# uthree/tinyvc

Measured on AMD Instinct MI355X. Metric: audio-samples/sec (16 kHz) end-to-end VC, higher is better.
Workload: dtype f32 (fp32 in / out / accumulate; channel contractions as two-term fp16 splits on v_mfma_f32_32x32x16_f16: 22-bit significands, three part-products per fp32 product)

## Files before the change

tinyvc_amd/csrc/api.hip:

```cpp
#include <atomic>
#include <cmath>
#include <mutex>

#include <cstdlib>

#include "knn_blob.h"
#include "tvc_common.h"

using namespace tvc;

static std::mutex g_blob_mu;
static std::map<const void*, int64_t> g_blobs;
constexpr size_t kMaxBlobRecords = 4096;
static void blob_record(const void* p, int64_t N) {
    std::lock_guard<std::mutex> lk(g_blob_mu);
    if (g_blobs.size() >= kMaxBlobRecords && !g_blobs.count(p)) g_blobs.clear();
    g_blobs[p] = N;
}
static void blob_forget(const void* p) {
    std::lock_guard<std::mutex> lk(g_blob_mu);
    g_blobs.erase(p);
}
static int blob_check(tvc_ctx* ctx, hipStream_t s, const void* p, int64_t N, const char* what) {
    {
// ... 12 lines not shown
        return fail(ctx, TVC_ERR_HIP, "%s: cannot read the prepared index's header", what);
    const int64_t n = ((int64_t)(unsigned)h[BLOB_W_N_HI] << 32) | (unsigned)h[BLOB_W_N_LO];
    if (h[BLOB_W_MAGIC] != BLOB_MAGIC || (h[BLOB_W_KIND] != KIND_F32 && h[BLOB_W_KIND] != KIND_F16))
        return fail(ctx, TVC_ERR_ARG, "%s: `prepared` is not a blob of tvc_knn_prepare_index_f32 / _f16", what);
    if (h[BLOB_W_VERSION] != tvc::kBlobVersion)
        return fail(ctx, TVC_ERR_ARG, "%s: the prepared index has format version %d, this library writes and reads version %d: prepare it again", what, h[BLOB_W_VERSION], tvc::kBlobVersion);
    if (n != N) return fail(ctx, TVC_ERR_ARG, "%s: this blob was prepared for N = %lld index vectors, the call says N = %lld", what, (long long)n, (long long)N);
    blob_record(p, N);
    return 0;
}

static int draw_under_capture(tvc_ctx* ctx, hipStream_t s, const float* noise_angle, const char* what) {
    if (noise_angle) return 0;
    hipStreamCaptureStatus cap = hipStreamCaptureStatusNone;
    if (hipStreamIsCapturing(s, &cap) == hipSuccess && cap != hipStreamCaptureStatusNone)
        return fail(ctx, TVC_ERR_STATE, "%s: noise_angle = NULL inside a stream capture would replay ONE seed's phases on every graph launch; pass noise_angle", what);
    return 0;
}

extern "C" {

int tvc_version(void) { return TVC_ABI_VERSION; }

int tvc_ctx_create(int hip_device, tvc_ctx** out) {
    if (!out) return TVC_ERR_ARG;
    *out = nullptr;
    int count = 0;
    if (hipGetDeviceCount(&count) != hipSuccess || hip_device < 0 || hip_device >= count) return TVC_ERR_HIP;
    tvc_ctx* c = new tvc_ctx();
    c->device = hip_device;
    {
        ArenaBuilder ab;
        pack_constants(c, &ab);
        if (hipSetDevice(hip_device) != hipSuccess ||
            hipMalloc((void**)&c->const_arena, ab.buf.size() * sizeof(float)) != hipSuccess ||
            hipMemcpy(c->const_arena, ab.buf.data(), ab.buf.size() * sizeof(float), hipMemcpyHostToDevice) != hipSuccess) {
            if (c->const_arena) (void)hipFree(c->const_arena);
            delete c;
            return TVC_ERR_HIP;
        }
        ab.resolve(c->const_arena);
    }
    if (hipDeviceGetAttribute(&c->ncu, hipDeviceAttributeMultiprocessorCount, hip_device) != hipSuccess) {
        tvc_ctx_destroy(c);
        return TVC_ERR_HIP;
    }
    int prio_least = 0, prio_greatest = 0;
    (void)hipDeviceGetStreamPriorityRange(&prio_least, &prio_greatest);
    if (hipStreamCreateWithPriority(&c->side, hipStreamNonBlocking, prio_least) != hipSuccess ||
        hipEventCreateWithFlags(&c->ev_fork, hipEventDisableTiming) != hipSuccess ||
        hipEventCreateWithFlags(&c->ev_join, hipEventDisableTiming) != hipSuccess ||
        hipEventCreateWithFlags(&c->ev_fork2, hipEventDisableTiming) != hipSuccess ||
        hipEventCreateWithFlags(&c->ev_join2, hipEventDisableTiming) != hipSuccess ||
        hipEventCreateWithFlags(&c->ev_amps, hipEventDisableTiming) != hipSuccess) {
        tvc_ctx_destroy(c);
        return TVC_ERR_HIP;
    }
    *out = c;
    return TVC_OK;
}

void tvc_ctx_destroy(tvc_ctx* ctx) {
    if (!ctx) return;
    (void)hipSetDevice(ctx->device);
    for (auto& r : ctx->regions) {
        if (r.a) (void)hipEventDestroy(r.a);
        if (r.b) (void)hipEventDestroy(r.b);
    }
    for (auto e : ctx->event_pool) (void)hipEventDestroy(e);
    if (ctx->ev_fork) (void)hipEventDestroy(ctx->ev_fork);
    if (ctx->ev_join) (void)hipEventDestroy(ctx->ev_join);
    if (ctx->ev_fork2) (void)hipEventDestroy(ctx->ev_fork2);
    if (ctx->ev_join2) (void)hipEventDestroy(ctx->ev_join2);
    if (ctx->ev_amps) (void)hipEventDestroy(ctx->ev_amps);
    if (ctx->side) (void)hipStreamDestroy(ctx->side);
    frontdoor_release(ctx);
    if (ctx->arena) (void)hipFree(ctx->arena);
    if (ctx->const_arena) (void)hipFree(ctx->const_arena);
    delete ctx;
}

const char* tvc_last_error(const tvc_ctx* ctx) { return ctx ? ctx->err : "null ctx"; }

int tvc_load_tensor(tvc_ctx* ctx, const char* key, const float* host_data, const int64_t* shape, int ndim) {
    if (!ctx || !key || !host_data || !shape || ndim < 1 || ndim > 4) return fail(ctx, TVC_ERR_ARG, "tvc_load_tensor: bad argument");
    size_t n = 1;
    HostTensor t;
    for (int i = 0; i < ndim; ++i) {
        if (shape[i] <= 0) return fail(ctx, TVC_ERR_ARG, "tvc_load_tensor(%s): bad shape", key);
        n *= (size_t)shape[i];
        t.shape.push_back(shape[i]);
    }
    t.data.assign(host_data, host_data + n);
    ctx->host[key] = std::move(t);
    ctx->enc_ready = ctx->dec_ready = false;
    return TVC_OK;
}

int tvc_set_pitch_table(tvc_ctx* ctx, const float* host_freqs, int n) {
    if (!ctx || !host_freqs || n != kPitchClasses) return fail(ctx, TVC_ERR_ARG, "pitch table must have %d entries", kPitchClasses);
    ctx->pitch_table.assign(host_freqs, host_freqs + n);
    ctx->enc_ready = ctx->dec_ready = false;
    return TVC_OK;
}

int tvc_finalize_weights(tvc_ctx* ctx) {
    if (!ctx) return TVC_ERR_ARG;
    ctx->enc_ready = ctx->dec_ready = false;
    ArenaBuilder ab;
    std::string missing_enc, missing_dec;
    pack_checkpoint(ctx, &ab, &missing_enc, &missing_dec);
    snprintf(ctx->enc_missing, sizeof(ctx->enc_missing), "%s", missing_enc.c_str());
    snprintf(ctx->dec_missing, sizeof(ctx->dec_missing), "%s", missing_dec.c_str());
    if (!missing_enc.empty() && !missing_dec.empty())
        return fail(ctx, TVC_ERR_STATE, "no complete checkpoint: encoder lacks %s; decoder lacks %s", missing_enc.c_str(), missing_dec.c_str());

    TVC_HIP(ctx, hipSetDevice(ctx->device));
    if (ctx->arena) {
        TVC_HIP(ctx, hipFree(ctx->arena));
        ctx->arena = nullptr;
    }
    ctx->arena_floats = ab.buf.size();
    TVC_HIP(ctx, hipMalloc((void**)&ctx->arena, ctx->arena_floats * sizeof(float)));
    TVC_HIP(ctx, hipMemcpy(ctx->arena, ab.buf.data(), ctx->arena_floats * sizeof(float), hipMemcpyHostToDevice));
    ab.resolve(ctx->arena);
    ctx->enc_ready = missing_enc.empty();
    ctx->dec_ready = missing_dec.empty();
// ... 1240 lines not shown
```

tinyvc_amd/csrc/decoder.hip:

```cpp
#include "conv3s.h"
#include "conv_s2.h"
#include "film_s2.h"
#include "gemm_s2.h"
#include "small_kernels.h"
#include "tvc_common.h"

namespace tvc {


__device__ __forceinline__ float div24k(float x) {
    const float r = 1.0f / 24000.0f;
    const float q0 = __fmul_rn(x, r);
    return fmaf(fmaf(-q0, 24000.0f, x), r, q0);
}

__device__ __forceinline__ double wave_incl_scan(double v, int lane) {
#pragma unroll
    for (int o = 1; o < 64; o <<= 1) {
        double u = __shfl_up(v, o);
        if (lane >= o) v += u;
    }
    return v;
}

// ... 171 lines not shown
    return launch_check(ctx, "harm_sums");
}

int run_dsp(tvc_ctx* ctx, hipStream_t s, Ws& ws, const float* f0, const float* amps, const float* kern, const float* angle, uint64_t seed, float* source, int B, int T,
            float* smax, double* csum, const DspFork* fk) {
    const long L = (long)T * kHop;
    if (!csum) csum = ws.get<double>((size_t)B * kHarm * T);
    float* frames = ws.get<float>((size_t)B * T * kNfft);
    const int NB = ctx->rag ? ctx->rag->B : B;
    const int Tg = ctx->rag ? ctx->rag->Tlong : T;
    float* smax_own = smax ? nullptr : ws.get<float>((size_t)NB);
    if (ws.dry) return 0;
    if (!smax) {
        smax = smax_own;
        TVC_HIP(ctx, hipMemsetAsync(smax, 0, (size_t)NB * sizeof(float), s));
    }
    RagDev rg;
    TVC_CHECK(rag_view(ctx, s, 1, 0, &rg, nullptr));
    const float scale_size = (float)T / (float)L;
    const float scale_amp = (float)(1.0 / (double)kHop);
    hipStream_t sh = s;
    if (fk) {
        sh = fk->side;
        TVC_HIP(ctx, hipStreamWaitEvent(sh, fk->amps_ready, 0));
    } else {
        TVC_CHECK(run_harm_sums(ctx, s, f0, csum, B, T));
    }
    hipLaunchKernelGGL(harm_synth_kernel, dim3((Tg + 3) / 4, NB), dim3(256), 0, sh, f0, amps, csum, source, T, scale_size, scale_amp, rg);
    TVC_CHECK(run_amax_rows(ctx, sh, amps, B, kHarm, T, smax));
    TVC_CHECK(run_noise_ifft(ctx, s, kern, angle, seed, frames, B, T, ctx->rag && angle));
    hipLaunchKernelGGL(noise_ola_kernel, dim3(grid_for((long)Tg * kHop / 4, 256, NB >= 32 ? 16 : 512 / NB), NB), dim3(256), 0, s, frames, source, B, T, smax, rg);
    return launch_check(ctx, "dsp");
}

static int plain_conv(tvc_ctx* ctx, hipStream_t s, const PackedW& w, const float* x, int B, int Cin, int len, int dil, float* y, const BfpSlots& bfp, int lin = 0,
                      float lscale = 0.f) {
    int rc = 0;
    if ((lin > 0 ? conv_s2_try<true>(&rc, ctx, s, w, x, B, Cin, len, dil, y, bfp, lin, lscale) : conv_s2_try<false>(&rc, ctx, s, w, x, B, Cin, len, dil, y, bfp)))
        return rc;
    if (lin > 0)
        return conv3s_launch<true, C3EpiBias<false>, false, true>(ctx, s, w, x, B, Cin, len, dil, C3EpiBias<false>{y, w.bias, nullptr, w.M, len}, bfp, nullptr, nullptr,
                                                                   nullptr, 0, lin, lscale);
    return conv3s_launch<true>(ctx, s, w, x, B, Cin, len, dil, C3EpiBias<false>{y, w.bias, nullptr, w.M, len}, bfp);
}

static int film_conv(tvc_ctx* ctx, hipStream_t s, const PackedW& w, const PackedW& fw, const FilmU& fu, const float* h, const float* cond, int B, int C, int len, int dil,
                     float* out, const float* bsc, const float* bsh, const float* res, int res_lin, float res_scale, const BfpSlots& bfp) {
    int rc = 0;
    if (rag_min_len(ctx, len) >= FS2::BN && film_s2_try(&rc, ctx, s, fu, h, cond, B, C, len, dil, out, res, res_lin, res_scale, bfp)) return rc;
    return conv3s_launch<true, C3EpiFilmFused, true>(ctx, s, w, h, B, C, len, dil, C3EpiFilmFused{out, w.bias, bsc, bsh, res, C, len, res_lin, res_scale}, bfp, &fw, &fw,
                                                     cond, C);
}

static int conv_film_half(tvc_ctx* ctx, hipStream_t s, const PackedW& ca, const PackedW& cb, const PackedW& fw, const FilmU& fu, const float* x, int lin, float lscale,
                          int da, int db, float* h, const float* cond, int B, int C, int len, float* out, const float* bsc, const float* bsh, const float* res,
                          int res_lin, float res_scale, const float* ma_in, float* mh, const float* mcond, float* mout) {
    const bool pre = rag_min_len(ctx, len) >= FS2::BN && fu.img && fu.C == C && fu.hb_w > 0.f && C % 96 == 0 && C <= 384 && ma_in && mcond && res && db >= 1 && db <= FS2::MAXD &&
                     (long)C * len * 4 < (1L << 32) && (res_lin <= 0 || (long)C * res_lin * 4 < (1L << 32));
    if (pre) {
        int rc = 0;
        const BfpSlots in{ma_in, nullptr, nullptr};
        const bool ok = lin > 0 ? conv_s2_try<true, true>(&rc, ctx, s, ca, x, B, C, len, da, h, in, lin, lscale, fu.hb_w, fu.hb_b)
                                : conv_s2_try<false, true>(&rc, ctx, s, ca, x, B, C, len, da, h, in, 0, 0.f, fu.hb_w, fu.hb_b);
        if (ok) {
            TVC_CHECK(rc);
            if (!film_s2_try(&rc, ctx, s, fu, h, cond, B, C, len, db, out, res, res_lin, res_scale, BfpSlots{ma_in, mcond, mout}, true, fu.hb_w, fu.hb_b))
                return fail(ctx, TVC_ERR_STATE, "filter_net: the FiLM conv refused the pre-split operand its producer wrote");
            return rc;
        }
    }
    TVC_CHECK(plain_conv(ctx, s, ca, x, B, C, len, da, h, BfpSlots{ma_in, nullptr, mh}, lin, lscale));
    return film_conv(ctx, s, cb, fw, fu, h, cond, B, C, len, db, out, bsc, bsh, res, res_lin, res_scale, BfpSlots{mh, mcond, mout});
}

static __global__ void g8_to_planar_kernel(const float* __restrict__ x, float* __restrict__ y, long B, long l, int C) {
    const long n = B * C * l;
    for (long i = blockIdx.x * (long)blockDim.x + threadIdx.x; i < n; i += (long)gridDim.x * blockDim.x) {
        const long t = i % l, bc = i / l, c = bc % C, b = bc / C;
        y[i] = x[((b * (C / 8) + c / 8) * l + t) * 8 + (c & 7)];
    }
}

static int filter_input_gemm(tvc_ctx* ctx, hipStream_t s, const float* content, const float* f0, float* x, int B, int T, const float* cmax) {
    EpiSumCond ep{x, ctx->flt_content_in.bias, nullptr, f0, nullptr, nullptr, ctx->flt_f_w, ctx->flt_f_b, 384, T, B * T};
    int rc = 0;
    if (!gemm_s2_try(&rc, ctx, s, ctx->flt_content_in, content, B, kSslDim, T, 0, ep, cmax)) rc = gemm_s_launch<2, 4, 2>(ctx, s, ctx->flt_content_in, content, B, kSslDim, T, 0, ep, cmax);
    return rc;
}

int run_filter(tvc_ctx* ctx, hipStream_t s, Ws& ws, const float* content, const float* f0,
               const float* energy, const float* source, float* wave, int B, int T, const FilterTaps* taps, const float* cmax, const float* smax, float* zeroed_slots, bool x_slot_set,
               float* x_pre, bool x_pre_filled) {
    const long L = (long)T * kHop;
    static const int ch[5] = {384, 192, 96, 48, 24};
    const long len_dn[5] = {L, L / 5, L / 20, L / 80, L / 240};
    float* skip[5];
    for (int i = 0; i < 5; ++i) skip[i] = ws.get<float>((size_t)B * ch[4 - i] * len_dn[i]);
    float* x = x_pre ? x_pre : ws.get<float>((size_t)B * ch[0] * T);
    float* xi_pre[5] = {nullptr, nullptr, nullptr, nullptr, nullptr};
    for (int i = 1; i <= 4; ++i) xi_pre[i] = ws.get<float>((size_t)B * ctx->downs[i - 1].cin * len_dn[i]);
    for (int i = 1; i < 4; ++i)
        if (len_dn[i] % ctx->downs[i].factor != 0 || (ctx->downs[i].factor == 4 && len_dn[i] % 4 != 0))
            return fail(ctx, TVC_ERR_ARG, "filter_net: level lengths must divide by the next Downsample factor");

    enum { S_CONTENT = 0, S_SRC, S_X, S_SKIP0, S_DH1 = S_SKIP0 + 5, S_DH2 = S_DH1 + 4, S_UHA = S_DH2 + 4, S_UX1 = S_UHA + 5, S_UHB = S_UX1 + 5, S_UXU = S_UHB + 5,
           S_LEV = S_UXU + 5, S_COUNT = S_LEV + 5 };
    const int NB = ctx->rag ? ctx->rag->B : B;
    static_assert(S_COUNT == kFilterSlots && S_X == kFilterSlotX, "tvc_common.h kFilterSlots / kFilterSlotX");
    float* slots = zeroed_slots ? zeroed_slots : ws.get<float>((size_t)S_COUNT * NB);
    auto slot = [&](int i) { return slots + (size_t)i * NB; };

    if (!ws.dry) {
        ProfScope ps(ctx, s, ws, "filter.in+down0");
        if (!zeroed_slots) TVC_HIP(ctx, hipMemsetAsync(slots, 0, (size_t)S_COUNT * NB * sizeof(float), s));
        if (!cmax) {
            TVC_CHECK(run_amax_rows(ctx, s, content, B, kSslDim, T, slot(S_CONTENT)));
            cmax = slot(S_CONTENT);
        }
        if (!smax) {
            TVC_CHECK(run_amax_rows(ctx, s, source, B, 16, L, slot(S_SRC)));
            TVC_CHECK(run_amax_rows(ctx, s, energy, B, 1, L, slot(S_SRC)));
            smax = slot(S_SRC);
        }
        if (!x_pre_filled) TVC_CHECK(filter_input_gemm(ctx, s, content, f0, x, B, T, cmax));
        if (!(zeroed_slots && x_slot_set)) TVC_CHECK(run_slot_affine(ctx, s, slot(S_X), cmax, 1, ctx->flt_in_bw, ctx->flt_in_bb, NB));
        TVC_CHECK(run_down0_split(ctx, s, ctx->flt_down0s, source, energy, skip[0], taps ? taps->skips[0] : nullptr, xi_pre[1], B, (int)L, smax, slot(S_SKIP0)));
    }
    for (int i = 1; i <= 4; ++i) {
        const DownW& d = ctx->downs[i - 1];
        const int len = (int)len_dn[i];
        size_t mk = ws.mark();
        float* xi = xi_pre[i];
        float* h1 = d.cin == 24 ? nullptr : ws.get<float>((size_t)B * d.cin * len);
        float* h2 = d.cin == 24 ? nullptr : ws.get<float>((size_t)B * d.cin * len);
        if (!ws.dry) {
            static const char* names[4] = {"filter.down1", "filter.down2", "filter.down3", "filter.down4"};
            ProfScope ps(ctx, s, ws, names[i - 1]);
            float* y2 = i < 4 ? xi_pre[i + 1] : nullptr;
            const int f2 = i < 4 ? ctx->downs[i].factor : 0;
            const float* mxi = slot(S_SKIP0 + i - 1);
            float *mh1 = slot(S_DH1 + i - 1), *mh2 = slot(S_DH2 + i - 1), *mout = slot(S_SKIP0 + i);
            if (d.cin == 24) {
                TVC_CHECK(run_down24_fused(ctx, s, d, xi, skip[i], y2, B, len, mxi, mout));
            } else {
                if (d.cin == 48) {
                    TVC_CHECK(run_conv48_pair(ctx, s, d.c1, d.c2, xi, 0, 0.f, nullptr, nullptr, nullptr, nullptr, h2, B, len, 1, 2, mxi, nullptr, mh2));
                } else {
                    TVC_CHECK(plain_conv(ctx, s, d.c1, xi, B, d.cin, len, 1, h1, BfpSlots{mxi, nullptr, mh1}));
                    TVC_CHECK(plain_conv(ctx, s, d.c2, h1, B, d.cin, len, 2, h2, BfpSlots{mh1, nullptr, mh2}));
                }
                TVC_CHECK((conv3s_launch<true, C3EpiBiasResConv>(ctx, s, d.c3, h2, B, d.cin, len, 4,
                                                                 C3EpiBiasResConv{{skip[i], d.c3res_bias, nullptr, d.cout, len, y2, f2}},
                                                                 BfpSlots{mh2, mxi, mout}, &d.res, nullptr, xi, d.cin)));
            }
        }
        ws.release(mk);
    }
    float* xlev[5];
    {
        long l = T;
        for (int i = 0; i < 5; ++i) {
            l *= ctx->ups[i].factor;
            xlev[i] = ws.get<float>((size_t)B * ctx->ups[i].cout * l);
        }
    }
    long len = T;
    const float* mx_in = slot(S_X);
    for (int i = 0; i < 5; ++i) {
        const UpW& u = ctx->ups[i];
        const int lin = (int)len;
        len *= u.factor;
        const int lo = (int)len, C = u.cin, nc = B * lo;
        const float* cond = skip[4 - i];
        const float* mcond = slot(S_SKIP0 + 4 - i);
        size_t mk = ws.mark();
        float* xu = ws.get<float>((size_t)B * C * lo);
        float* h = ws.get<float>((size_t)B * C * lo);
        float* x1 = ws.get<float>((size_t)B * C * lo);
        if (!ws.dry && C == 24) {
            ProfScope ps(ctx, s, ws, "filter.up4+out");
            TVC_CHECK(run_up24_split(ctx, s, u, x, cond, ctx->down0_bw, ctx->down0_bb, x1, wave, B, lo, mx_in, smax, slot(S_UX1 + i)));
        } else if (!ws.dry) {
            static const char* names[4] = {"filter.up0", "filter.up1", "filter.up2", "filter.up3"};
            ProfScope ps(ctx, s, ws, names[i]);
            const float lscale = (float)(1.0 / (double)u.factor);
            for (int half = 0; half < 2; ++half) {
                const PackedW& ca = half ? u.c3 : u.c1;
                const PackedW& cb = half ? u.c4 : u.c2;
                const PackedW& fw = half ? u.film2 : u.film1;
                const float* bsc = fw.bias;
                const float* bsh = fw.bias + C;
                const int da = half ? 9 : 1, db = half ? 27 : 3;
                float* xout = half ? xu : x1;
                const float* ma_in = half ? slot(S_UX1 + i) : mx_in;
                float* mh = slot((half ? S_UHB : S_UHA) + i);
                float* mout = slot((half ? S_UXU : S_UX1) + i);
                if (C == 48) {
                    if (half == 0) {
                        TVC_CHECK(run_conv48_pair(ctx, s, ca, cb, x, lin, lscale, &fw, bsc, bsh, cond, xout, B, lo, da, db, ma_in, mcond, mout));
                    } else {
                        TVC_CHECK(run_conv48s(ctx, s, ca, x1, nullptr, nullptr, nullptr, nullptr, nullptr, h, B, lo, da, ma_in, nullptr, mh));
                        TVC_CHECK(run_conv48s(ctx, s, cb, h, &fw, bsc, bsh, cond, x1, nullptr, B, lo, db, mh, mcond, slot(S_LEV + i), &u.c5, xlev[i]));
                    }
                } else if (half == 0) {
                    TVC_CHECK(conv_film_half(ctx, s, ca, cb, fw, u.fu1, x, lin, lscale, da, db, h, cond, B, C, lo, xout, bsc, bsh, x, lin, lscale, ma_in, mh, mcond, mout));
                } else {
                    TVC_CHECK(conv_film_half(ctx, s, ca, cb, fw, u.fu2, x1, 0, 0.f, da, db, h, cond, B, C, lo, xout, bsc, bsh, x1, 0, 0.f, ma_in, mh, mcond, mout));
                }
            }
            if (C != 48) {
                EpiBias<ACT_NONE, false> ep{xlev[i], u.c5.bias, nullptr, u.cout, lo, nc, (long)u.cout * lo, 0, slot(S_LEV + i), slot(S_UXU + i), u.c5_bw, u.c5_bb, NB};
                if (u.cout == 48) {
                    EpiBiasG8 eg{xlev[i], u.c5.bias, u.cout, lo, nc, slot(S_LEV + i), slot(S_UXU + i), u.c5_bw, u.c5_bb, NB};
                    TVC_CHECK((gemm_s_launch<2, 4, 2>(ctx, s, u.c5, xu, B, C, lo, 0, eg, slot(S_UXU + i))));
                } else if (u.c5.MT6 % 3 == 0) TVC_CHECK((gemm_s_launch<3, 4, 1>(ctx, s, u.c5, xu, B, C, lo, 0, ep, slot(S_UXU + i))));
                else TVC_CHECK((gemm_s_launch<2, 4, 2>(ctx, s, u.c5, xu, B, C, lo, 0, ep, slot(S_UXU + i))));
            }
        }
        ws.release(mk);
        x = xlev[i];
        mx_in = slot(S_LEV + i);
    }
    if (!ws.dry && taps) {
        for (int i = 1; i < 5; ++i)
            if (taps->skips[i] && i == 1)
                hipLaunchKernelGGL(g8_to_planar_kernel, dim3(grid_for((long)B * 48 * len_dn[1])), dim3(256), 0, s, skip[1], taps->skips[1], (long)B, len_dn[1], 48);
            else if (taps->skips[i])
                TVC_HIP(ctx, hipMemcpyAsync(taps->skips[i], skip[i], (size_t)B * ch[4 - i] * len_dn[i] * sizeof(float), hipMemcpyDeviceToDevice, s));
        long l = T;
        for (int i = 0; i < 4; ++i) {
            l *= ctx->ups[i].factor;
            if (taps->ups[i] && ctx->ups[i].cout <= 48)
                hipLaunchKernelGGL(g8_to_planar_kernel, dim3(grid_for((long)B * ctx->ups[i].cout * l)), dim3(256), 0, s, xlev[i], taps->ups[i], (long)B, l, ctx->ups[i].cout);
            else if (taps->ups[i])
                TVC_HIP(ctx, hipMemcpyAsync(taps->ups[i], xlev[i], (size_t)B * ctx->ups[i].cout * l * sizeof(float), hipMemcpyDeviceToDevice, s));
        }
    }
    return ws.dry ? 0 : launch_check(ctx, "filter_net");
}

int run_decoder(tvc_ctx* ctx, hipStream_t s, Ws& ws, const float* content, const float* f0,
                const float* energy, const float* angle, uint64_t seed, float* wave, float* amps_out,
                float* kernel_out, float* source_out, int B, int T, const float* content_bound, const float* energy_bound,
                int content_bound_stride) {
    const long L = (long)T * kHop;
    float* amps = amps_out ? amps_out : ws.get<float>((size_t)B * kHarm * T);
    float* kern = kernel_out ? kernel_out : ws.get<float>((size_t)B * kBins * T);
    float* source = source_out ? source_out : ws.get<float>((size_t)B * 16 * L);
    const int NB = ctx->rag ? ctx->rag->B : B;
    float* cmax = ws.get<float>((size_t)(3 + kFilterSlots) * NB);
    float* smax = cmax + NB;
    float* xmax = smax + NB;
    float* fslots = xmax + NB;
    float* x0 = ws.get<float>((size_t)B * 384 * T);
    double* csum = ws.get<double>((size_t)B * kHarm * T);
    if (!ws.dry) {
        TVC_CHECK(run_slot_prep(ctx, s, cmax, (3 + kFilterSlots) * NB, content_bound ? cmax : nullptr, content_bound, content_bound_stride, 1.f, 0.f, energy_bound ? smax : nullptr,
                                energy_bound, 1, 1.f, 0.f, content_bound ? fslots + (size_t)kFilterSlotX * NB : nullptr, ctx->flt_in_bw, ctx->flt_in_bb,
                                NB));
        if (!content_bound) TVC_CHECK(run_amax_rows(ctx, s, content, B, kSslDim, T, cmax));
        if (!energy_bound) TVC_CHECK(run_amax_rows(ctx, s, energy, B, 1, L, smax));
    }
    SideFork fk(ctx, s);
    if (wave) TVC_CHECK(fk.fork(ws, ctx->ev_fork2, ctx->ev_join2));
    if (fk.forked()) {
        TVC_CHECK(run_harm_sums(ctx, fk.side, f0, csum, B, T));
        ProfScope ps(ctx, fk.side, ws, "filter_net.input@side");
        TVC_CHECK(filter_input_gemm(ctx, fk.side, content, f0, x0, B, T, cmax));
    }
    size_t mk = ws.mark();
    {
        ProfScope ps(ctx, s, ws, "source_net");
        TVC_CHECK(run_source_net(ctx, s, ws, content, f0, energy, amps, kern, B, T, cmax, xmax, fk.forked() ? ctx->ev_amps : nullptr));
    }
    ws.release(mk);
    if (!wave && !source_out) return 0;
    {
        ProfScope ps(ctx, s, ws, "dsp");
        const DspFork df{fk.side, ctx->ev_amps};
        TVC_CHECK(run_dsp(ctx, s, ws, f0, amps, kern, angle, seed, source, B, T, smax, csum, fk.forked() ? &df : nullptr));
        TVC_CHECK(fk.join());
    }
    ws.release(mk);
    if (!wave) return 0;
    ProfScope ps(ctx, s, ws, "filter_net");
    TVC_CHECK(run_filter(ctx, s, ws, content, f0, energy, source, wave, B, T, nullptr, cmax, smax, fslots, content_bound != nullptr, x0, fk.forked()));
    ws.release(mk);
    return 0;
}

}
```

tinyvc_amd/csrc/tvc_common.h:

```cpp
#pragma once
#include <hip/hip_runtime.h>

#include <atomic>
#include <cstdarg>
#include <cstdint>
#include <cstdio>
#include <cstring>
#include <map>
#include <string>
#include <vector>

#include "../../include/tinyvc_hip.h"
#include "ragged.h"

namespace tvc {

constexpr int kSampleRate = 24000;
constexpr int kNfft = 1920;
constexpr int kHop = 480;
constexpr int kBins = 961;
constexpr int kSslDim = 768;
constexpr int kSslCh = 384;
constexpr int kPitchCh = 128;
constexpr int kPitchClasses = 512;
// ... 52 lines not shown
    const float* s24c1 = nullptr;
    const float* s24c2 = nullptr;
    const float* s24c3r = nullptr;
    float b1_w = 0.f, b1_b = 0.f, b2_w = 0.f, b2_b = 0.f;
    int cin = 0, cout = 0, factor = 1;
};
struct FilmU {
    static constexpr int TAB_BIAS = 0, TAB_SCALE = 1, TAB_BSC = 2, TAB_BSH = 3, TAB_SSC = 4, TAB_SSH = 5;
    const float* img = nullptr;
    const float* tab = nullptr;
    int C = 0;
    float hb_w = 0.f, hb_b = 0.f;
};
struct UpW {
    PackedW c1, c2, c3, c4, c5, film1, film2;
    FilmU fu1, fu2;
    const float* s24a = nullptr;
    const float* s24b = nullptr;
    float c5_bw = 0.f, c5_bb = 0.f;
    int cin = 0, cout = 0, factor = 1;
};

struct HostTensor {
    std::vector<float> data;
    std::vector<int64_t> shape;
};

struct ArenaBuilder {
    std::vector<float> buf;
    std::vector<std::pair<const float**, size_t>> fix;
    size_t put(const float** slot, const float* v, size_t n);
    size_t put(const float** slot, const std::vector<float>& v) { return put(slot, v.data(), v.size()); }
    void resolve(const float* arena) const {
        for (auto& f : fix) *f.first = arena + f.second;
    }
};

}

struct tvc_prof_region {
    std::string name;
    hipEvent_t a = nullptr, b = nullptr;
};

struct tvc_ctx {
    int device = 0;
    int ncu = 0;
    int profiling = 0;
    std::vector<tvc_prof_region> regions;
    std::vector<hipEvent_t> event_pool;
    hipStream_t side = nullptr;
    hipEvent_t ev_fork = nullptr, ev_join = nullptr;
    hipEvent_t ev_fork2 = nullptr, ev_join2 = nullptr, ev_amps = nullptr;
    tvc::RagHost* rag = nullptr;
    int rag_batch_frames = 0;
    int index_assign_chunk = 0;
    bool enc_ready = false, dec_ready = false;
    char enc_missing[160] = {0}, dec_missing[160] = {0};
    std::map<std::string, tvc::HostTensor> host;
    std::vector<float> pitch_table;
    float* arena = nullptr;
    float* const_arena = nullptr;
    size_t arena_floats = 0;
    char err[512] = {0};

    const float* fft_tw960 = nullptr;
    const float* fft_tw1920 = nullptr;
    const float* fft_hann = nullptr;
    const float* pitch_freq = nullptr;
    const float* sola_part = nullptr;
    const float* dn_win = nullptr;
    const float* dn_tw320 = nullptr;
    const float* dn_tw640 = nullptr;

    tvc::PackedW enc_in;
    const float* ssl_ln_g = nullptr;
    const float* ssl_ln_b = nullptr;
    const float* pit_ln_g = nullptr;
    const float* pit_ln_b = nullptr;
    tvc::ConvNeXtW ssl_mid[6], pit_mid[4], src_mid[3];
    tvc::PackedW ssl_out, pit_out;
    tvc::PackedW src_content_in, src_to_amps, src_to_kernel;
    const float* src_e_w = nullptr;
    const float* src_e_b = nullptr;
    const float* src_f_w = nullptr;
    const float* src_f_b = nullptr;
    tvc::PackedW flt_content_in;
    const float* flt_down0s = nullptr;
    float down0_bw = 0.f, down0_bb = 0.f;
    float flt_in_bw = 0.f, flt_in_bb = 0.f;
    const float* flt_f_w = nullptr;
    const float* flt_f_b = nullptr;
    tvc::DownW downs[4];
    tvc::UpW ups[5];
};

namespace tvc {

inline int fail(tvc_ctx* ctx, int code, const char* fmt, ...) {
    if (ctx) {
        va_list ap;
        va_start(ap, fmt);
        vsnprintf(ctx->err, sizeof(ctx->err), fmt, ap);
        va_end(ap);
    }
    return code;
// ... 22 lines not shown
    T* get(size_t n) {
        size_t bytes = (n * sizeof(T) + 255) & ~size_t(255);
        size_t o = off;
        off += bytes;
        if (off > peak) peak = off;
        if (dry) return (T*)(uintptr_t)256;
        return (T*)(base + o);
    }
    size_t mark() const { return off; }
    void release(size_t m) { off = m; }
};

struct ProfScope {
    tvc_ctx* ctx;
    hipStream_t s;
    int idx = -1;
    ProfScope(tvc_ctx* c, hipStream_t st, const Ws& ws, const char* name) : ctx(c), s(st) {
        if (!c || !c->profiling || ws.dry) return;
        if (c->profiling == 2 && std::strncmp(name, "filter_net", 10) != 0) return;
        tvc_prof_region r;
        r.name = name;
        auto take = [&](hipEvent_t* e) {
            if (!c->event_pool.empty()) {
                *e = c->event_pool.back();
                c->event_pool.pop_back();
                return true;
            }
            return hipEventCreate(e) == hipSuccess;
        };
        if (!take(&r.a) || !take(&r.b)) return;
        (void)hipEventRecord(r.a, s);
        c->regions.push_back(r);
        idx = (int)c->regions.size() - 1;
    }
    ~ProfScope() {
        if (idx >= 0) (void)hipEventRecord(ctx->regions[idx].b, s);
    }
};

struct SideFork {
    tvc_ctx* ctx;
    hipStream_t s, side;
    hipEvent_t ev_join = nullptr;
    bool ended = false;
    SideFork(tvc_ctx* c, hipStream_t st) : ctx(c), s(st), side(st) {}
    bool forked() const { return ev_join != nullptr; }
    int fork(const Ws& ws, hipEvent_t ev_fork, hipEvent_t join) {
        hipStreamCaptureStatus cap = hipStreamCaptureStatusNone;
        if (ws.dry || !ctx->side || !ev_fork || !join || hipStreamIsCapturing(s, &cap) != hipSuccess || cap != hipStreamCaptureStatusNone) return 0;
        TVC_HIP(ctx, hipEventRecord(ev_fork, s));
        TVC_HIP(ctx, hipStreamWaitEvent(ctx->side, ev_fork, 0));
        side = ctx->side;
        ev_join = join;
        return 0;
    }
    int end() {
        if (forked() && !ended) TVC_HIP(ctx, hipEventRecord(ev_join, side));
        ended = true;
        return 0;
    }
    hipError_t record_and_wait() {
        hipEvent_t e = ev_join;
        ev_join = nullptr;
        const hipError_t r = e && !ended ? hipEventRecord(e, side) : hipSuccess;
        return e && r == hipSuccess ? hipStreamWaitEvent(s, e, 0) : r;
    }
    int join() { TVC_HIP(ctx, record_and_wait()); return 0; }
    ~SideFork() { (void)record_and_wait(); }
};

inline int launch_check(tvc_ctx* ctx, const char* what) {
    hipError_t e = hipGetLastError();
    if (e != hipSuccess) return fail(ctx, TVC_ERR_HIP, "launch %s: %s", what, hipGetErrorString(e));
    return 0;
}

template <auto... K>
int lds_optin(tvc_ctx* ctx, int bytes, const char* what) {
    static std::atomic<bool> ready_dev[64];
    std::atomic<bool>& ready = ready_dev[ctx->device & 63];
    if (ready.load(std::memory_order_acquire)) return 0;
    for (const void* k : {(const void*)K...}) {
        const hipError_t e = hipFuncSetAttribute(k, hipFuncAttributeMaxDynamicSharedMemorySize, bytes);
        if (e != hipSuccess) return fail(ctx, TVC_ERR_HIP, "%s setup: %s", what, hipGetErrorString(e));
    }
    ready.store(true, std::memory_order_release);
    return 0;
}

void pack_constants(tvc_ctx*, ArenaBuilder*);
void pack_checkpoint(tvc_ctx*, ArenaBuilder*, std::string* missing_enc, std::string* missing_dec);

int run_stft(tvc_ctx*, hipStream_t, Ws&, const float* wav, float* spec, int B, int64_t L);
int run_stft_fft(tvc_ctx*, hipStream_t, const float* wav, float* spec, int B, int64_t L);
int run_noise_ifft(tvc_ctx*, hipStream_t, const float* kern, const float* angle, uint64_t seed, float* frames, int B, int T, bool angle_padded = false);
int run_energy(tvc_ctx*, hipStream_t, Ws&, const float* wav, float* energy, int B, int64_t L, float* emax = nullptr, float* spec_bound = nullptr,
               float* zero = nullptr, int nz = 0);
int run_knn_amax_rows(tvc_ctx*, hipStream_t, const std::vector<const float*>& blobs, float* out);
int run_slot_affine(tvc_ctx*, hipStream_t, float* out, const float* in, int in_stride, float a, float c, int n);
int run_slot_prep(tvc_ctx*, hipStream_t, float* zero, int nz, float* o1, const float* in1, int s1, float a1, float c1, float* o2, const float* in2, int s2, float a2,
                  float c2, float* o3, float a3, float c3, int n);
constexpr int kBlobMagic = 0x54564B4E, kBlobVersion = 2;
constexpr int kFilterSlotX = 2;
constexpr int kFilterSlots = 41;
int run_encoder(tvc_ctx*, hipStream_t, Ws&, const float* spec, float* ssl, float* f0,
                float* logits, int B, int T, const float* spec_bound = nullptr, float* zeroed_slots = nullptr,
// ... 40 lines not shown
};
struct ConvertCall {
    const float* wav = nullptr;
    float* wave = nullptr;
    int B = 0;
    int64_t L = 0;
    const int64_t* lens = nullptr;
    ConvertIndex index;
    float shift = 0.f;
    const float* shifts = nullptr;
    const float* angle = nullptr;
    uint64_t seed = 0;
    const float* target_f0 = nullptr;
    float* shift_out = nullptr;
    const PitchTrackState* track = nullptr;
    const float* alpha = nullptr;
    const float* protect = nullptr;
    const tvc_pitch_path* path = nullptr;
};
int convert_impl(tvc_ctx*, hipStream_t, Ws&, const ConvertCall& c);
int run_knn_topk(tvc_ctx*, hipStream_t, Ws&, const float* src, const float* prepared, int64_t N,
                 float* sims_out, int64_t* idx_out, int B, int T);
int run_knn_general(tvc_ctx*, hipStream_t, Ws&, const float* src, const float* index, int64_t N, int k, int metric, float* out, int64_t* idx_out,
                    float* val_out, int B, int T);
int run_knn_slots(tvc_ctx*, hipStream_t, const float* prepared, int64_t N, const int64_t* idx, float* slots, int64_t nslots);
int run_knn_finish(tvc_ctx*, hipStream_t, const float* slots, float* out, int B, int T);
int run_shift(tvc_ctx*, hipStream_t, const float* f0, float* out, int64_t n, float semitones);
struct PitchRow {
    int start, len, idx;
    float offset;
};
int run_pitch_match(tvc_ctx*, hipStream_t, const float* f0, const std::vector<PitchRow>& rows, const float* target, float* median_out, int* voiced_out,
                    float* shift_out, float* f0s);
int run_pitch_track(tvc_ctx*, hipStream_t, const float* f0, int S, int T, const PitchTrackState& t, const float* target, float offset,
                    const float* offsets, float* median_out, int64_t* count_out, float* shift_out, float* f0s);
constexpr int kPitchPathMaxBand = TVC_PITCH_PATH_MAX_BAND, kPitchPathMaxRefine = TVC_PITCH_PATH_MAX_REFINE;
struct PitchPathRow {
    int start, len;
    float shift;
};
size_t pitch_path_ws_bytes(int64_t columns);
int pitch_path_check(const tvc_pitch_path& p, char* why, size_t why_bytes);
int run_pitch_path(tvc_ctx*, hipStream_t, const float* logits, long S, const std::vector<PitchPathRow>& rows, const tvc_pitch_path& p, uint16_t* bp, float* f0,
                   float* f0s, int* path_out, float* score_out);
int run_uniform_to_angle(tvc_ctx*, hipStream_t, float* u, int64_t n);
int run_decoder(tvc_ctx*, hipStream_t, Ws&, const float* content, const float* f0,
                const float* energy, const float* angle, uint64_t seed, float* wave, float* amps_out,
                float* kernel_out, float* source_out, int B, int T, const float* content_bound = nullptr, const float* energy_bound = nullptr,
                int content_bound_stride = 0);
struct FilterTaps {
    float* skips[5] = {nullptr, nullptr, nullptr, nullptr, nullptr};
    float* ups[4] = {nullptr, nullptr, nullptr, nullptr};
};
int run_filter(tvc_ctx*, hipStream_t, Ws&, const float* content, const float* f0, const float* energy,
               const float* source, float* wave, int B, int T, const FilterTaps* taps = nullptr, const float* cmax = nullptr, const float* smax = nullptr,
               float* zeroed_slots = nullptr, bool x_slot_set = false, float* x_pre = nullptr, bool x_pre_filled = false);
struct DspFork {
    hipStream_t side;
    hipEvent_t amps_ready;
};
int run_dsp(tvc_ctx*, hipStream_t, Ws&, const float* f0, const float* amps, const float* kern, const float* angle, uint64_t seed, float* source, int B, int T,
            float* smax = nullptr, double* csum = nullptr, const DspFork* fk = nullptr);
int sola_geometry(int block, int cross, int search, int delay, int64_t* min_ly, int* latency_min, int* latency_max, char* why, size_t why_bytes);
int run_sola(tvc_ctx*, hipStream_t, const float* y, float* sola_buf, const float* fade_in, float* out, int32_t* shift_out,
             int S, int64_t Ly, int block, int cross, int search, int delay, int use_pv);
int run_stream_push(tvc_ctx* ctx, hipStream_t s, float* buf, const float* blocks, int S, int n, int m);
constexpr int kGateMaxSub = 4096, kGateMaxSubFrame = 1 << 16, kGateMaxCount = 1 << 20;
struct StreamGate {
    int block, sub, look, hold, attack, release;
    float hysteresis_db, range_db;
    const float* threshold_db;
    int32_t* open;
    int32_t* hold_state;
    float* gain;
    float* level_db;
};
int stream_gate_geometry(int block, int sub, int look, int hold, int attack, int release, int* nsub, int* look_samples, char* why, size_t why_bytes);
int run_stream_gate(tvc_ctx*, hipStream_t, const float* x, int64_t n, int64_t base, const int32_t* shift, const float* y, float* out, int S, const StreamGate& g);
constexpr int kLoudnessTile = 64, kLoudnessChunk = 512, kLoudnessMaxSmooth = 32, kLoudnessMaxSubFrame = 1 << 16;
constexpr int kLoudnessMaxBlockSub = 4096;
constexpr int64_t kLoudnessMaxLength = (int64_t)1 << 40;
constexpr int kLoudnessLenRows = 384;
struct LoudnessLens {
    int64_t v[kLoudnessLenRows];
};
struct LoudnessConst {
    double floor, lo, hi;
};
struct StreamLoudness {
    int block, sub, smooth;
    const float* share;
    double* src_ring;
    double* out_ring;
    int64_t* frames;
    float* gain;
    float* gain_db;
};
int loudness_geometry(int64_t length, int sub, int smooth, bool stream_block, int64_t* nsub, int* window, int* tile, char* why, size_t why_bytes);
int loudness_constants(float floor_db, float boost_db, float cut_db, LoudnessConst* c, char* why, size_t why_bytes);
int run_loudness_match(tvc_ctx*, hipStream_t, const float* x, const float* y, float* out, int B, int64_t L, const int64_t* lengths, const float* share, int sub,
                       int smooth, const LoudnessConst& c, float* gains);
int run_stream_loudness(tvc_ctx*, hipStream_t, const float* x, int64_t n, int64_t base, const int32_t* shift, const float* y, float* out, int S,
                        const StreamLoudness& g, const LoudnessConst& c, float* gains);
constexpr int kLimiterTile = 512, kLimiterEdges = (kLimiterTile + 1 + 255) / 256, kLimiterChunk = 512, kLimiterMaxRelease = 4096, kLimiterMaxSubFrame = 1 << 16;
constexpr int kLimiterMaxBlock = 1 << 30;
constexpr int64_t kLimiterMaxLength = (int64_t)1 << 40;
struct StreamLimiter {
    int block, sub;
    const float* ceiling;
// ... 63 lines not shown
```

Measured before the change: 740.1 million.

## Run first up-block conv on side stream overlapping down path

Splits the first half of the filter's up0 conv+FiLM block into a producer conv and a FiLM step. The first conv (which depends only on the filter input) now runs on the side stream after the input GEMM, overlapping with the down-path work on the main stream. The main stream joins before the FiLM conv. This adds a partial join event after the DSP stage, moves slot-affine and rag tile setup ahead of the fork, and carries a cross-stream ordering risk on the shared slot and h0 buffers.

```diff
diff --git a/tinyvc_amd/csrc/api.hip b/tinyvc_amd/csrc/api.hip
--- a/tinyvc_amd/csrc/api.hip
+++ b/tinyvc_amd/csrc/api.hip
@@ -88,7 +88,8 @@
         hipEventCreateWithFlags(&c->ev_join, hipEventDisableTiming) != hipSuccess ||
         hipEventCreateWithFlags(&c->ev_fork2, hipEventDisableTiming) != hipSuccess ||
         hipEventCreateWithFlags(&c->ev_join2, hipEventDisableTiming) != hipSuccess ||
-        hipEventCreateWithFlags(&c->ev_amps, hipEventDisableTiming) != hipSuccess) {
+        hipEventCreateWithFlags(&c->ev_amps, hipEventDisableTiming) != hipSuccess ||
+        hipEventCreateWithFlags(&c->ev_src, hipEventDisableTiming) != hipSuccess) {
         tvc_ctx_destroy(c);
         return TVC_ERR_HIP;
     }
@@ -109,6 +110,7 @@
     if (ctx->ev_fork2) (void)hipEventDestroy(ctx->ev_fork2);
     if (ctx->ev_join2) (void)hipEventDestroy(ctx->ev_join2);
     if (ctx->ev_amps) (void)hipEventDestroy(ctx->ev_amps);
+    if (ctx->ev_src) (void)hipEventDestroy(ctx->ev_src);
     if (ctx->side) (void)hipStreamDestroy(ctx->side);
     frontdoor_release(ctx);
     if (ctx->arena) (void)hipFree(ctx->arena);
diff --git a/tinyvc_amd/csrc/decoder.hip b/tinyvc_amd/csrc/decoder.hip
--- a/tinyvc_amd/csrc/decoder.hip
+++ b/tinyvc_amd/csrc/decoder.hip
@@ -247,26 +247,45 @@
                                                      cond, C);
 }
 
-static int conv_film_half(tvc_ctx* ctx, hipStream_t s, const PackedW& ca, const PackedW& cb, const PackedW& fw, const FilmU& fu, const float* x, int lin, float lscale,
-                          int da, int db, float* h, const float* cond, int B, int C, int len, float* out, const float* bsc, const float* bsh, const float* res,
-                          int res_lin, float res_scale, const float* ma_in, float* mh, const float* mcond, float* mout) {
-    const bool pre = rag_min_len(ctx, len) >= FS2::BN && fu.img && fu.C == C && fu.hb_w > 0.f && C % 96 == 0 && C <= 384 && ma_in && mcond && res && db >= 1 && db <= FS2::MAXD &&
+static int half_first(tvc_ctx* ctx, hipStream_t s, const PackedW& ca, const FilmU& fu, const float* x, int lin, float lscale, int da, int db, float* h, int B, int C, int len,
+                      const float* res, int res_lin, const float* ma_in, float* mh, const float* mcond, bool* pre) {
+    *pre = false;
+    const bool can = rag_min_len(ctx, len) >= FS2::BN && fu.img && fu.C == C && fu.hb_w > 0.f && C % 96 == 0 && C <= 384 && ma_in && mcond && res && db >= 1 && db <= FS2::MAXD &&
                      (long)C * len * 4 < (1L << 32) && (res_lin <= 0 || (long)C * res_lin * 4 < (1L << 32));
-    if (pre) {
+    if (can) {
         int rc = 0;
         const BfpSlots in{ma_in, nullptr, nullptr};
         const bool ok = lin > 0 ? conv_s2_try<true, true>(&rc, ctx, s, ca, x, B, C, len, da, h, in, lin, lscale, fu.hb_w, fu.hb_b)
                                 : conv_s2_try<false, true>(&rc, ctx, s, ca, x, B, C, len, da, h, in, 0, 0.f, fu.hb_w, fu.hb_b);
         if (ok) {
-            TVC_CHECK(rc);
-            if (!film_s2_try(&rc, ctx, s, fu, h, cond, B, C, len, db, out, res, res_lin, res_scale, BfpSlots{ma_in, mcond, mout}, true, fu.hb_w, fu.hb_b))
-                return fail(ctx, TVC_ERR_STATE, "filter_net: the FiLM conv refused the pre-split operand its producer wrote");
+            *pre = rc == 0;
             return rc;
         }
     }
-    TVC_CHECK(plain_conv(ctx, s, ca, x, B, C, len, da, h, BfpSlots{ma_in, nullptr, mh}, lin, lscale));
+    return plain_conv(ctx, s, ca, x, B, C, len, da, h, BfpSlots{ma_in, nullptr, mh}, lin, lscale);
+}
+
+static int half_film(tvc_ctx* ctx, hipStream_t s, const PackedW& cb, const PackedW& fw, const FilmU& fu, int db, const float* h, const float* cond, int B, int C, int len,
+                     float* out, const float* bsc, const float* bsh, const float* res, int res_lin, float res_scale, const float* ma_in, const float* mh, const float* mcond,
+                     float* mout, bool pre) {
+    if (pre) {
+        int rc = 0;
+        if (!film_s2_try(&rc, ctx, s, fu, h, cond, B, C, len, db, out, res, res_lin, res_scale, BfpSlots{ma_in, mcond, mout}, true, fu.hb_w, fu.hb_b))
+            return fail(ctx, TVC_ERR_STATE, "filter_net: the FiLM conv refused the pre-split operand its producer wrote");
+        return rc;
+    }
     return film_conv(ctx, s, cb, fw, fu, h, cond, B, C, len, db, out, bsc, bsh, res, res_lin, res_scale, BfpSlots{mh, mcond, mout});
 }
+
+static int conv_film_half(tvc_ctx* ctx, hipStream_t s, const PackedW& ca, const PackedW& cb, const PackedW& fw, const FilmU& fu, const float* x, int lin, float lscale,
+                          int da, int db, float* h, const float* cond, int B, int C, int len, float* out, const float* bsc, const float* bsh, const float* res,
+                          int res_lin, float res_scale, const float* ma_in, float* mh, const float* mcond, float* mout) {
+    bool pre = false;
+    TVC_CHECK(half_first(ctx, s, ca, fu, x, lin, lscale, da, db, h, B, C, len, res, res_lin, ma_in, mh, mcond, &pre));
+    return half_film(ctx, s, cb, fw, fu, db, h, cond, B, C, len, out, bsc, bsh, res, res_lin, res_scale, ma_in, mh, mcond, mout, pre);
+}
+
+constexpr int kHalfDil[2][2] = {{1, 3}, {9, 27}};
 
 static __global__ void g8_to_planar_kernel(const float* __restrict__ x, float* __restrict__ y, long B, long l, int C) {
     const long n = B * C * l;
@@ -285,13 +304,18 @@
 
 int run_filter(tvc_ctx* ctx, hipStream_t s, Ws& ws, const float* content, const float* f0,
                const float* energy, const float* source, float* wave, int B, int T, const FilterTaps* taps, const float* cmax, const float* smax, float* zeroed_slots, bool x_slot_set,
-               float* x_pre, bool x_pre_filled) {
+               const FilterFront* front) {
     const long L = (long)T * kHop;
     static const int ch[5] = {384, 192, 96, 48, 24};
     const long len_dn[5] = {L, L / 5, L / 20, L / 80, L / 240};
     float* skip[5];
     for (int i = 0; i < 5; ++i) skip[i] = ws.get<float>((size_t)B * ch[4 - i] * len_dn[i]);
-    float* x = x_pre ? x_pre : ws.get<float>((size_t)B * ch[0] * T);
+    float* x = front ? front->x0 : ws.get<float>((size_t)B * ch[0] * T);
+    const UpW& u0 = ctx->ups[0];
+    const int lo0 = T * u0.factor;
+    float* h0 = front ? front->h0 : ws.get<float>((size_t)B * u0.cin * lo0);
+    SideFork* fk = front && front->fk && front->fk->forked() ? front->fk : nullptr;
+    bool pre0 = false;
     float* xi_pre[5] = {nullptr, nullptr, nullptr, nullptr, nullptr};
     for (int i = 1; i <= 4; ++i) xi_pre[i] = ws.get<float>((size_t)B * ctx->downs[i - 1].cin * len_dn[i]);
     for (int i = 1; i < 4; ++i)
@@ -304,6 +328,10 @@
     static_assert(S_COUNT == kFilterSlots && S_X == kFilterSlotX, "tvc_common.h kFilterSlots / kFilterSlotX");
     float* slots = zeroed_slots ? zeroed_slots : ws.get<float>((size_t)S_COUNT * NB);
     auto slot = [&](int i) { return slots + (size_t)i * NB; };
+    auto up0_first = [&](hipStream_t st) {
+        return half_first(ctx, st, u0.c1, u0.fu1, x, T, (float)(1.0 / (double)u0.factor), kHalfDil[0][0], kHalfDil[0][1], h0, B, u0.cin, lo0, x, T, slot(S_X), slot(S_UHA),
+                          slot(S_SKIP0 + 4), &pre0);
+    };
 
     if (!ws.dry) {
         ProfScope ps(ctx, s, ws, "filter.in+down0");
@@ -317,8 +345,16 @@
             TVC_CHECK(run_amax_rows(ctx, s, energy, B, 1, L, slot(S_SRC)));
             smax = slot(S_SRC);
         }
-        if (!x_pre_filled) TVC_CHECK(filter_input_gemm(ctx, s, content, f0, x, B, T, cmax));
+        if (fk && !(zeroed_slots && x_slot_set)) return fail(ctx, TVC_ERR_STATE, "filter_net: a forked front needs its slots prepared in front of the fork");
+        if (!fk) TVC_CHECK(filter_input_gemm(ctx, s, content, f0, x, B, T, cmax));
         if (!(zeroed_slots && x_slot_set)) TVC_CHECK(run_slot_affine(ctx, s, slot(S_X), cmax, 1, ctx->flt_in_bw, ctx->flt_in_bb, NB));
+        if (fk) {
+            {
+                ProfScope ps(ctx, fk->side, ws, "filter_net.input@side");
+                TVC_CHECK(up0_first(fk->side));
+            }
+            TVC_CHECK(fk->end());
+        }
         TVC_CHECK(run_down0_split(ctx, s, ctx->flt_down0s, source, energy, skip[0], taps ? taps->skips[0] : nullptr, xi_pre[1], B, (int)L, smax, slot(S_SKIP0)));
     }
     for (int i = 1; i <= 4; ++i) {
@@ -370,7 +406,7 @@
         const float* mcond = slot(S_SKIP0 + 4 - i);
         size_t mk = ws.mark();
         float* xu = ws.get<float>((size_t)B * C * lo);
-        float* h = ws.get<float>((size_t)B * C * lo);
+        float* h = i == 0 ? h0 : ws.get<float>((size_t)B * C * lo);
         float* x1 = ws.get<float>((size_t)B * C * lo);
         if (!ws.dry && C == 24) {
             ProfScope ps(ctx, s, ws, "filter.up4+out");
@@ -385,7 +421,7 @@
                 const PackedW& fw = half ? u.film2 : u.film1;
                 const float* bsc = fw.bias;
                 const float* bsh = fw.bias + C;
-                const int da = half ? 9 : 1, db = half ? 27 : 3;
+                const int da = kHalfDil[half][0], db = kHalfDil[half][1];
                 float* xout = half ? xu : x1;
                 const float* ma_in = half ? slot(S_UX1 + i) : mx_in;
                 float* mh = slot((half ? S_UHB : S_UHA) + i);
@@ -397,6 +433,10 @@
                         TVC_CHECK(run_conv48s(ctx, s, ca, x1, nullptr, nullptr, nullptr, nullptr, nullptr, h, B, lo, da, ma_in, nullptr, mh));
                         TVC_CHECK(run_conv48s(ctx, s, cb, h, &fw, bsc, bsh, cond, x1, nullptr, B, lo, db, mh, mcond, slot(S_LEV + i), &u.c5, xlev[i]));
                     }
+                } else if (half == 0 && i == 0) {
+                    if (fk) TVC_CHECK(fk->join());
+                    else TVC_CHECK(up0_first(s));
+                    TVC_CHECK(half_film(ctx, s, cb, fw, u.fu1, db, h, cond, B, C, lo, xout, bsc, bsh, x, lin, lscale, ma_in, mh, mcond, mout, pre0));
                 } else if (half == 0) {
                     TVC_CHECK(conv_film_half(ctx, s, ca, cb, fw, u.fu1, x, lin, lscale, da, db, h, cond, B, C, lo, xout, bsc, bsh, x, lin, lscale, ma_in, mh, mcond, mout));
                 } else {
@@ -448,6 +488,7 @@
     float* xmax = smax + NB;
     float* fslots = xmax + NB;
     float* x0 = ws.get<float>((size_t)B * 384 * T);
+    float* h0 = ws.get<float>((size_t)B * ctx->ups[0].cin * T * ctx->ups[0].factor);
     double* csum = ws.get<double>((size_t)B * kHarm * T);
     if (!ws.dry) {
         TVC_CHECK(run_slot_prep(ctx, s, cmax, (3 + kFilterSlots) * NB, content_bound ? cmax : nullptr, content_bound, content_bound_stride, 1.f, 0.f, energy_bound ? smax : nullptr,
@@ -455,9 +496,15 @@
                                 NB));
         if (!content_bound) TVC_CHECK(run_amax_rows(ctx, s, content, B, kSslDim, T, cmax));
         if (!energy_bound) TVC_CHECK(run_amax_rows(ctx, s, energy, B, 1, L, smax));
+        if (!content_bound && wave) TVC_CHECK(run_slot_affine(ctx, s, fslots + (size_t)kFilterSlotX * NB, cmax, 1, ctx->flt_in_bw, ctx->flt_in_bb, NB));
+        if (wave && ctx->rag) {
+            RagDev rd;
+            TVC_CHECK(rag_tiles(ctx, s, B, (long)T * ctx->ups[0].factor, CS2::BN, &rd, nullptr, "filter_net front"));
+        }
     }
     SideFork fk(ctx, s);
     if (wave) TVC_CHECK(fk.fork(ws, ctx->ev_fork2, ctx->ev_join2));
+    const FilterFront front{&fk, x0, h0};
     if (fk.forked()) {
         TVC_CHECK(run_harm_sums(ctx, fk.side, f0, csum, B, T));
         ProfScope ps(ctx, fk.side, ws, "filter_net.input@side");
@@ -474,12 +521,12 @@
         ProfScope ps(ctx, s, ws, "dsp");
         const DspFork df{fk.side, ctx->ev_amps};
         TVC_CHECK(run_dsp(ctx, s, ws, f0, amps, kern, angle, seed, source, B, T, smax, csum, fk.forked() ? &df : nullptr));
-        TVC_CHECK(fk.join());
+        TVC_CHECK(fk.join_so_far(ctx->ev_src));
     }
     ws.release(mk);
     if (!wave) return 0;
     ProfScope ps(ctx, s, ws, "filter_net");
-    TVC_CHECK(run_filter(ctx, s, ws, content, f0, energy, source, wave, B, T, nullptr, cmax, smax, fslots, content_bound != nullptr, x0, fk.forked()));
+    TVC_CHECK(run_filter(ctx, s, ws, content, f0, energy, source, wave, B, T, nullptr, cmax, smax, fslots, true, &front));
     ws.release(mk);
     return 0;
 }
diff --git a/tinyvc_amd/csrc/tvc_common.h b/tinyvc_amd/csrc/tvc_common.h
--- a/tinyvc_amd/csrc/tvc_common.h
+++ b/tinyvc_amd/csrc/tvc_common.h
@@ -128,6 +128,7 @@
     hipStream_t side = nullptr;
     hipEvent_t ev_fork = nullptr, ev_join = nullptr;
     hipEvent_t ev_fork2 = nullptr, ev_join2 = nullptr, ev_amps = nullptr;
+    hipEvent_t ev_src = nullptr;
     tvc::RagHost* rag = nullptr;
     int rag_batch_frames = 0;
     int index_assign_chunk = 0;
@@ -256,6 +257,12 @@
         TVC_HIP(ctx, hipStreamWaitEvent(ctx->side, ev_fork, 0));
         side = ctx->side;
         ev_join = join;
+        return 0;
+    }
+    int join_so_far(hipEvent_t ev) {
+        if (!forked()) return 0;
+        TVC_HIP(ctx, hipEventRecord(ev, side));
+        TVC_HIP(ctx, hipStreamWaitEvent(s, ev, 0));
         return 0;
     }
     int end() {
@@ -402,9 +409,13 @@
     float* skips[5] = {nullptr, nullptr, nullptr, nullptr, nullptr};
     float* ups[4] = {nullptr, nullptr, nullptr, nullptr};
 };
+struct FilterFront {
+    SideFork* fk;
+    float *x0, *h0;
+};
 int run_filter(tvc_ctx*, hipStream_t, Ws&, const float* content, const float* f0, const float* energy,
                const float* source, float* wave, int B, int T, const FilterTaps* taps = nullptr, const float* cmax = nullptr, const float* smax = nullptr,
-               float* zeroed_slots = nullptr, bool x_slot_set = false, float* x_pre = nullptr, bool x_pre_filled = false);
+               float* zeroed_slots = nullptr, bool x_slot_set = false, const FilterFront* front = nullptr);
 struct DspFork {
     hipStream_t side;
     hipEvent_t amps_ready;
```

Measured after the change: 751.4 million (median of 6 runs). 1.02x the previous value.
